# Soldann/MORB_SLAM

Hardware: AMD Instinct MI355X
Metric: stereo frames/sec ORB extract+match (752x480, 1200 feat = BASELINE configs[1]) (higher is better)
Workload: dtype u8; 1 GPU; BASELINE configs[1]: EuRoC-shaped stereo 752x480, 1200 feat: ORBextractor x2 + ComputeStereoMatches + ComputeBoW (synthetic k=10 L=6 vocabulary) + SearchByBoW vs previous frame; steps_in_flight=2, extract_streams=1, parallelism=frames dealt round-robin over 1 GPU(s)

## Files before the change

morb_slam_amd/csrc/matcher.hip:

```cpp
#include <hip/hip_runtime.h>

#include <algorithm>
#include <cstdlib>
#include <cstring>
#include <memory>
#include <vector>

#include "common.h"
#include "internal_abi.h"
#include "wave.h"
#include "extractor_internal.h"

using namespace morb;

namespace {

constexpr int TH_HIGH = 100, TH_LOW = 50, HISTO_LENGTH = 30;

struct Desc { uint32_t w[8]; };

__device__ __forceinline__ Desc load_desc(const uint8_t* p) {
  Desc d;
  const uint4* q = reinterpret_cast<const uint4*>(p);
  const uint4 a = q[0], b = q[1];
// ... 31 lines not shown
__global__ __launch_bounds__(256) void k_hamming_pairs(const uint8_t* __restrict__ a, const uint8_t* __restrict__ b, int n,
                                                       int* __restrict__ out) {
  const int i = blockIdx.x * 256 + threadIdx.x;
  if (i < n) out[i] = hamming(load_desc(a + (size_t)i * 32), load_desc(b + (size_t)i * 32));
}

__global__ __launch_bounds__(256) void k_knn2(const uint8_t* __restrict__ q, const int* __restrict__ nqv, int qPitch,
                                              const uint8_t* __restrict__ t, const int* __restrict__ ntv, int tPitch,
                                              const int* __restrict__ qOffv, const int* __restrict__ tOffv,
                                              int* __restrict__ idx, int* __restrict__ dist) {
  __shared__ uint4 tile[256 * 2];
  const int prob = blockIdx.y;
  const int qOff = qOffv ? qOffv[prob] : 0, tOff = tOffv ? tOffv[prob] : 0;
  const int nq = nqv[prob] - qOff, nt = ntv[prob] - tOff;
  const int i = blockIdx.x * 256 + threadIdx.x;
  const uint8_t* qb = q + ((size_t)prob * qPitch + qOff) * 32;
  const uint8_t* tb = t + ((size_t)prob * tPitch + tOff) * 32;
  if ((int)blockIdx.x * 256 >= nq) return;
  Desc d;
  if (i < nq) d = load_desc(qb + (size_t)i * 32);
  unsigned long long k1 = ~0ull, k2 = ~0ull;
  for (int j0 = 0; j0 < nt; j0 += 256) {
    const int j = j0 + threadIdx.x;
    if (j < nt) {
      const uint4* src = reinterpret_cast<const uint4*>(tb + (size_t)j * 32);
      tile[threadIdx.x * 2] = src[0];
      tile[threadIdx.x * 2 + 1] = src[1];
    }
    __syncthreads();
    const int m = nt - j0 < 256 ? nt - j0 : 256;
    if (i < nq) {
      for (int jj = 0; jj < m; ++jj) {
        const uint4 a = tile[jj * 2], b = tile[jj * 2 + 1];
        const int s = __popc(d.w[0] ^ a.x) + __popc(d.w[1] ^ a.y) + __popc(d.w[2] ^ a.z) + __popc(d.w[3] ^ a.w) +
                      __popc(d.w[4] ^ b.x) + __popc(d.w[5] ^ b.y) + __popc(d.w[6] ^ b.z) + __popc(d.w[7] ^ b.w);
        top2_insert(k1, k2, ((unsigned long long)s << 32) | (unsigned)(j0 + jj));
      }
    }
    __syncthreads();
  }
  if (i < nq) {
    const size_t o = ((size_t)prob * qPitch + i) * 2;
    idx[o] = k1 == ~0ull ? -1 : (int)(k1 & 0xFFFFFFFFu);
    dist[o] = k1 == ~0ull ? -1 : (int)(k1 >> 32);
    idx[o + 1] = k2 == ~0ull ? -1 : (int)(k2 & 0xFFFFFFFFu);
    dist[o + 1] = k2 == ~0ull ? -1 : (int)(k2 >> 32);
  }
}

__host__ __device__ inline int sm_lk_for(int nframes) { return nframes <= 2 ? 4 : nframes <= 8 ? 8 : nframes <= 32 ? 16 : 32; }
constexpr int SM_BAND = 16;
constexpr int SM_MAXB = 256;
struct StereoGeom {
  unsigned long long pyrOff[16], pyrImg[16];
  int pstride[16], w[16];
  float scale[16], invScale[16];
  int nRows;
};
struct RightKp { uint32_t band; float x; };
constexpr int SM_LIST = 4;
constexpr int SM_KQ = 8;
constexpr int SM_PCAP = 512;
constexpr int SM_PATCH = 11 * 12 + 11 * 24;
static_assert(4 * SM_PATCH <= SM_PCAP * 4, "four keypoints' patches reuse the pair list");
#define WAVE_SYNC() do { __builtin_amdgcn_fence(__ATOMIC_SEQ_CST, "workgroup"); __builtin_amdgcn_wave_barrier(); } while (0)
__device__ __forceinline__ uint32_t load_u32_unaligned(const uint8_t* p) { uint32_t v; __builtin_memcpy(&v, p, 4); return v; }

struct StereoRec { int band, list, bytes; };
__host__ __device__ inline StereoRec stereo_rec(int cap) {
  StereoRec r;
  r.band = (cap * (int)sizeof(RightKp) + 15) & ~15;
  r.list = r.band + (((SM_MAXB + 2) * 4 + 15) & ~15);
  r.bytes = r.list + ((SM_LIST * cap * 2 + 15) & ~15);
  return r;
}
__global__ __launch_bounds__(1024) void k_stereo_prep(const StereoGeom sg, const morb_keypoint* __restrict__ kps, const int* __restrict__ count,
                                                     int cap, uint8_t* __restrict__ rec) {
  extern __shared__ __align__(16) uint8_t smem[];
  const StereoRec ro = stereo_rec(cap);
  RightKp* tab = reinterpret_cast<RightKp*>(smem);
  int* bandStart = reinterpret_cast<int*>(smem + ro.band);
  uint16_t* list = reinterpret_cast<uint16_t*>(smem + ro.list);
  int* bandFill = reinterpret_cast<int*>(smem + ro.bytes);
  const int f = blockIdx.x, tid = threadIdx.x, lane = tid & 63, NT = blockDim.x;
  const int imgR = 2 * f + 1, NR = count[imgR];
  const int nRows = sg.nRows;
  const int nBands = (nRows + SM_BAND - 1) / SM_BAND;
  const bool banded = nBands <= SM_MAXB;
  for (int i = tid; i < SM_MAXB + 2; i += NT) { bandStart[i] = 0; if (i < SM_MAXB) bandFill[i] = 0; }
  __syncthreads();
  for (int iR = tid; iR < NR; iR += NT) {
    const morb_keypoint kpR = kps[(size_t)imgR * cap + iR];
    const float r = 2.0f * sg.scale[kpR.octave & 15];
    const int maxr = (int)ceilf(kpR.y + r), minr = (int)floorf(kpR.y - r);
    const int lo = min(max(minr, -4095), 4095) + 4096, hi = min(max(maxr, -4095), 4095) + 4096;
    RightKp t;
    t.band = (uint32_t)lo | ((uint32_t)hi << 14) | ((uint32_t)kpR.octave << 28); t.x = kpR.x;
    tab[iR] = t;
    if (banded && maxr >= 0 && minr < nRows)
      for (int bnd = max(minr, 0) / SM_BAND; bnd <= min(maxr, nRows - 1) / SM_BAND; ++bnd) atomicAdd(&bandStart[bnd + 1], 1);
  }
  __syncthreads();
  if (tid < 64) {
    int c[4], sum = 0;
#pragma unroll
    for (int k = 0; k < 4; ++k) { c[k] = bandStart[1 + tid * 4 + k]; sum += c[k]; }
    int inc = sum;
#pragma unroll
    for (int d = 1; d < 64; d <<= 1) { const int o = __shfl_up(inc, d, 64); if (lane >= d) inc += o; }
    int acc = inc - sum;
#pragma unroll
    for (int k = 0; k < 4; ++k) { acc += c[k]; bandStart[1 + tid * 4 + k] = acc; }
    if (tid == 63) bandStart[SM_MAXB + 1] = acc;
  }
  __syncthreads();
  const int listTotal = bandStart[SM_MAXB + 1];
  if (banded && listTotal <= SM_LIST * cap) {
    for (int iR = tid; iR < NR; iR += NT) {
      const RightKp t = tab[iR];
      const int minr = (int)(t.band & 0x3FFF) - 4096, maxr = (int)((t.band >> 14) & 0x3FFF) - 4096;
      if (maxr >= 0 && minr < nRows)
        for (int bnd = max(minr, 0) / SM_BAND; bnd <= min(maxr, nRows - 1) / SM_BAND; ++bnd)
          list[bandStart[bnd] + atomicAdd(&bandFill[bnd], 1)] = (uint16_t)iR;
    }
  }
  __syncthreads();
  const uint4* src = reinterpret_cast<const uint4*>(smem);
  uint4* dst = reinterpret_cast<uint4*>(rec + (size_t)f * ro.bytes);
  for (int i = tid; i < (ro.bytes >> 4); i += NT) dst[i] = src[i];
}

__global__ __launch_bounds__(256) void k_stereo_match(const StereoGeom sg, const uint8_t* __restrict__ pyr,
                                                      const morb_keypoint* __restrict__ kps,
                                                      const uint8_t* __restrict__ desc, const int* __restrict__ count,
                                                      int cap, float mbf, float mb,
                                                      float* __restrict__ uRight, float* __restrict__ depth,
                                                      int* __restrict__ sadDist, int SM_LK, const uint8_t* __restrict__ rec) {
  extern __shared__ __align__(16) uint8_t smem[];
  uint4* dLAll = reinterpret_cast<uint4*>(smem);
  unsigned long long* bestAll = reinterpret_cast<unsigned long long*>(dLAll + 4 * SM_KQ * 2);
  uint32_t* pairsAll = reinterpret_cast<uint32_t*>(bestAll + 4 * SM_KQ);
  uint8_t* recL = reinterpret_cast<uint8_t*>(pairsAll + 4 * SM_PCAP);
  const StereoRec ro = stereo_rec(cap);
  const RightKp* tab = reinterpret_cast<const RightKp*>(recL);
  const int* bandStart = reinterpret_cast<const int*>(recL + ro.band);
  const uint16_t* list = reinterpret_cast<const uint16_t*>(recL + ro.list);
  const int f = blockIdx.y, tid = threadIdx.x, lane = tid & 63, wv = tid >> 6;
  const int imgL = 2 * f, imgR = 2 * f + 1;
  const int NL = count[imgL], NR = count[imgR];
  const int iL0 = blockIdx.x * SM_LK;
  if (iL0 >= cap) return;
  const int nRows = sg.nRows;
  const int nBands = (nRows + SM_BAND - 1) / SM_BAND;
  const bool banded = nBands <= SM_MAXB;
  const uint8_t* recG = rec + (size_t)f * ro.bytes;
  const int listTotal = reinterpret_cast<const int*>(recG + ro.band)[SM_MAXB + 1];
  const bool useBands = banded && listTotal <= SM_LIST * cap;
  if (iL0 < NL) {
    const uint4* src = reinterpret_cast<const uint4*>(recG);
    uint4* dst = reinterpret_cast<uint4*>(recL);
    const int nTab = (NR * (int)sizeof(RightKp) + 15) >> 4, nBand = ((SM_MAXB + 2) * 4 + 15) >> 4, nList = useBands ? (listTotal * 2 + 15) >> 4 : 0;
    for (int i = tid; i < nTab; i += 256) dst[i] = src[i];
    for (int i = tid; i < nBand; i += 256) dst[(ro.band >> 4) + i] = src[(ro.band >> 4) + i];
    for (int i = tid; i < nList; i += 256) dst[(ro.list >> 4) + i] = src[(ro.list >> 4) + i];
  }
  __syncthreads();
#if defined(MORB_STEREO_STOP) && MORB_STEREO_STOP == 1
  return;
#endif
  const int KQ = SM_LK / 4;
  uint32_t* pairs = pairsAll + wv * SM_PCAP;
  uint4* dLs = dLAll + wv * (SM_KQ * 2);
  unsigned long long* bestL = bestAll + wv * SM_KQ;
  const uint64_t lt = lane == 0 ? 0ull : (~0ull >> (64 - lane));
  const float maxD = mbf / mb;
  float myX = 0.f, myY = 0.f;
  int myOct = 0;
  if (lane < KQ) {
    const int iL = iL0 + lane * 4 + wv;
    if (iL < NL) { const morb_keypoint k = kps[(size_t)imgL * cap + iL]; myX = k.x; myY = k.y; myOct = k.octave; }
  }
  if (lane < 2 * KQ) {
    const int iL = iL0 + (lane >> 1) * 4 + wv;
    uint4 v = make_uint4(0, 0, 0, 0);
    if (iL < NL) v = reinterpret_cast<const uint4*>(desc + ((size_t)imgL * cap + iL) * 32)[lane & 1];
    dLs[lane] = v;
  }
  if (lane < SM_KQ) bestL[lane] = ~0ull;
  WAVE_SYNC();

  auto flush = [&](int n) {
    WAVE_SYNC();
    for (int c0 = 0; c0 < n; c0 += 64) {
      const int c = c0 + lane;
      const bool act = c < n;
      const uint32_t pr = pairs[act ? c : n - 1];
      const int q = (int)(pr >> 16), jR = (int)(pr & 0xFFFFu);
      unsigned long long key = ~0ull;
      if (act) {
        Desc dL;
        const uint4 a = dLs[2 * q], b = dLs[2 * q + 1];
        dL.w[0] = a.x; dL.w[1] = a.y; dL.w[2] = a.z; dL.w[3] = a.w; dL.w[4] = b.x; dL.w[5] = b.y; dL.w[6] = b.z; dL.w[7] = b.w;
        const int d = hamming(dL, load_desc(desc + ((size_t)imgR * cap + jR) * 32));
        if (d < TH_HIGH) key = ((unsigned long long)d << 32) | (unsigned)jR;
      }
      if (cap <= 65536) {
        static_assert(SM_KQ <= 256 && TH_HIGH <= 256, "the packed key holds (SM_KQ - 1 - q) in 8 bits, a distance < TH_HIGH in 8 bits and the right index in 16");
        uint32_t ck = ((uint32_t)(SM_KQ - 1 - q) << 24) | (key == ~0ull ? 0xFFFFFFu : (((uint32_t)(key >> 32) << 16) | (uint32_t)(key & 0xFFFFu)));
        MORB_DPP_SCAN(ck, 0xFFFFFFFFu, morbwave::op_umin);
        const int qn = (int)(pairs[c + 1 < n ? c + 1 : n - 1] >> 16);
        const bool runEnd = act && (c == n - 1 || lane == 63 || qn != q);
        const uint32_t m24 = ck & 0xFFFFFFu;
        if (runEnd && m24 != 0xFFFFFFu) {
          const unsigned long long m = ((unsigned long long)(m24 >> 16) << 32) | (m24 & 0xFFFFu);
          if (m < bestL[q]) bestL[q] = m;
        }
      } else {
        const int qlo = __builtin_amdgcn_readfirstlane(q), qhi = __builtin_amdgcn_readlane(q, 63);
        for (int qq = qlo; qq <= qhi; ++qq) {
          const unsigned long long m = wave_min_u64(q == qq ? key : ~0ull);
          if (lane == 0 && m < bestL[qq]) bestL[qq] = m;
        }
      }
    }
    WAVE_SYNC();
  };
  {
    int n = 0;
    for (int q = 0; q < KQ; ++q) {
      const int iL = iL0 + q * 4 + wv;
      if (iL >= NL) break;
      const int levelL = __builtin_amdgcn_readlane(myOct, q);
      const float vL = __builtin_bit_cast(float, __builtin_amdgcn_readlane(__builtin_bit_cast(int, myY), q));
      const float uL = __builtin_bit_cast(float, __builtin_amdgcn_readlane(__builtin_bit_cast(int, myX), q));
      const int row = (int)vL;
      const float minU = uL - maxD, maxU = uL - 0.f;
      if (!(row >= 0 && row < nRows && !(maxU < 0))) continue;
      const int e0 = useBands ? bandStart[row / SM_BAND] : 0, e1 = useBands ? bandStart[row / SM_BAND + 1] : NR;
      for (int j0 = e0; j0 < e1; j0 += 64) {
        const int ei = j0 + lane;
        bool ok = false;
        int iR = 0;
        if (ei < e1) {
          iR = useBands ? (int)list[ei] : ei;
          const RightKp t = tab[iR];
          const int minr = (int)(t.band & 0x3FFF) - 4096, maxr = (int)((t.band >> 14) & 0x3FFF) - 4096, oct = (int)(t.band >> 28);
          ok = row >= minr && row <= maxr && !(oct < levelL - 1 || oct > levelL + 1) && t.x >= minU && t.x <= maxU;
        }
        const uint64_t m = __ballot(ok);
        if (ok) pairs[n + __popcll(m & lt)] = ((uint32_t)q << 16) | (uint32_t)iR;
        n += __popcll(m);
        if (n > SM_PCAP - 64) { flush(n); n = 0; }
      }
    }
    if (n) flush(n);
  }
#if defined(MORB_STEREO_STOP) && MORB_STEREO_STOP == 2
  return;
#endif
  bool cDo = false;
  float cUL = 0.f, cUR0 = 0.f;
  int cLvl = 0, cPs = 0;
  unsigned long long cOffL = 0, cOffR = 0;
  if (lane < KQ) {
    const int iL = iL0 + lane * 4 + wv;
    if (iL < NL) {
      const unsigned long long best = bestL[lane];
      const int bestDist = best == ~0ull ? TH_HIGH : (int)(best >> 32);
      if (bestDist < (TH_HIGH + TH_LOW) / 2) {
        const int bestIdxR = (int)(best & 0xFFFFFFFFu);
        const int levelL = myOct;
        const float vL = myY, uL = myX;
        const float uR0 = tab[bestIdxR].x;
        const float sf = sg.invScale[levelL & 15];
        const float scaleduL = roundf(uL * sf), scaledvL = roundf(vL * sf), scaleduR0 = roundf(uR0 * sf);
        const unsigned long long pyrOff = sg.pyrOff[levelL & 15], pyrImg = sg.pyrImg[levelL & 15];
        const int pstride = sg.pstride[levelL & 15], w = sg.w[levelL & 15];
        const float iniu = scaleduR0 + 5 - 5, endu = scaleduR0 + 5 + 5 + 1;
        if (!(iniu < 0 || endu >= (float)w)) {
          cDo = true; cUL = uL; cUR0 = scaleduR0; cLvl = levelL; cPs = pstride;
          cOffL = pyrOff + (size_t)imgL * pyrImg + (size_t)(kPyrPad + (int)scaledvL) * pstride + kPyrPad + (int)scaleduL;
          cOffR = pyrOff + (size_t)imgR * pyrImg + (size_t)(kPyrPad + (int)scaledvL) * pstride + kPyrPad + (int)scaleduR0;
        }
      }
    }
  }
  int pRow[2], pCol[2], pLds[2];
  bool pLeft[2], pAct[2];
#pragma unroll
  for (int j = 0; j < 2; ++j) {
    const int t = lane + 64 * j;
    pAct[j] = t < 99; pLeft[j] = t < 33;
    if (t < 33) {
      const int r = t / 3, c4 = (t - r * 3) * 4;
      pRow[j] = r - 5; pCol[j] = c4 - 5; pLds[j] = r * 12 + c4;
    } else {
      const int t2 = min(t, 98) - 33, r = t2 / 6, c4 = (t2 - r * 6) * 4;
      pRow[j] = r - 5; pCol[j] = c4 - 10; pLds[j] = 11 * 12 + r * 24 + c4;
    }
  }
  const uint64_t doMask = __ballot(cDo);
  const uint32_t cOffLlo = (uint32_t)cOffL, cOffLhi = (uint32_t)(cOffL >> 32), cOffRlo = (uint32_t)cOffR, cOffRhi = (uint32_t)(cOffR >> 32);
  uint8_t* patch = reinterpret_cast<uint8_t*>(pairs);
  int rS = -1, rInc = 0;
  float rD1 = 0.f, rD3 = 0.f;
  const int dy = min(lane & 15, 10);
  for (int q0 = 0; q0 < KQ; q0 += 4) {
    if (((doMask >> q0) & 15ull) == 0) continue;
    uint32_t pv[4][2];
#pragma unroll
    for (int k = 0; k < 4; ++k) {
      const int q = q0 + k;
      pv[k][0] = pv[k][1] = 0;
      if ((doMask >> q) & 1ull) {
        const unsigned long long oL = ((unsigned long long)(uint32_t)__builtin_amdgcn_readlane((int)cOffLhi, q) << 32) | (uint32_t)__builtin_amdgcn_readlane((int)cOffLlo, q);
        const unsigned long long oR = ((unsigned long long)(uint32_t)__builtin_amdgcn_readlane((int)cOffRhi, q) << 32) | (uint32_t)__builtin_amdgcn_readlane((int)cOffRlo, q);
        const int ps = __builtin_amdgcn_readlane(cPs, q);
#pragma unroll
        for (int j = 0; j < 2; ++j)
          if (pAct[j]) pv[k][j] = load_u32_unaligned(pyr + (pLeft[j] ? oL : oR) + (ptrdiff_t)pRow[j] * ps + pCol[j]);
      }
    }
    WAVE_SYNC();
#pragma unroll
    for (int k = 0; k < 4; ++k) {
      if (!((doMask >> (q0 + k)) & 1ull)) continue;
#pragma unroll
      for (int j = 0; j < 2; ++j)
        if (pAct[j]) *reinterpret_cast<uint32_t*>(patch + k * SM_PATCH + pLds[j]) = pv[k][j];
    }
    WAVE_SYNC();
#pragma unroll
    for (int k = 0; k < 4; ++k) {
      const int q = q0 + k;
      if (!((doMask >> q) & 1ull)) continue;
      const uint8_t* Lp = patch + k * SM_PATCH;
      const uint8_t* Rp = Lp + 11 * 12;
      const uint32_t l0 = *reinterpret_cast<const uint32_t*>(Lp + dy * 12), l1 = *reinterpret_cast<const uint32_t*>(Lp + dy * 12 + 4),
                     l2 = *reinterpret_cast<const uint32_t*>(Lp + dy * 12 + 8) & 0x00FFFFFFu;
      uint32_t bestKey = 0xFFFFFFFFu;
      int sums[12];
#pragma unroll
      for (int r = 0; r < 3; ++r) {
        const int sh = min(r * 4 + (lane >> 4), 10);
        const uint8_t* rp = Rp + dy * 24 + (sh & ~3);
        const uint32_t w0 = *reinterpret_cast<const uint32_t*>(rp), w1 = *reinterpret_cast<const uint32_t*>(rp + 4),
                       w2 = *reinterpret_cast<const uint32_t*>(rp + 8), w3 = *reinterpret_cast<const uint32_t*>(rp + 12);
        const uint32_t bsh = (uint32_t)(sh & 3);
        const uint32_t r0 = __builtin_amdgcn_alignbyte(w1, w0, bsh), r1 = __builtin_amdgcn_alignbyte(w2, w1, bsh),
                       r2 = __builtin_amdgcn_alignbyte(w3, w2, bsh) & 0x00FFFFFFu;
        int sv = (int)__builtin_amdgcn_sad_u8(l2, r2, __builtin_amdgcn_sad_u8(l1, r1, __builtin_amdgcn_sad_u8(l0, r0, 0u)));
        if ((lane & 15) > 10) sv = 0;
        sv += __builtin_amdgcn_update_dpp(0, sv, 0x111, 0xf, 0xf, true);
        sv += __builtin_amdgcn_update_dpp(0, sv, 0x112, 0xf, 0xf, true);
        sv += __builtin_amdgcn_update_dpp(0, sv, 0x114, 0xf, 0xf, true);
        sv += __builtin_amdgcn_update_dpp(0, sv, 0x118, 0xf, 0xf, true);
#pragma unroll
        for (int j = 0; j < 4; ++j) {
          sums[r * 4 + j] = __builtin_amdgcn_readlane(sv, 16 * j + 15);
          if (r * 4 + j < 11) {
            const uint32_t key = ((uint32_t)sums[r * 4 + j] << 4) | (uint32_t)(r * 4 + j);
            bestKey = key < bestKey ? key : bestKey;
          }
        }
      }
      const int bestS = (int)(bestKey >> 4), bi = (int)(bestKey & 15u);
      int s1 = 0, s3 = 0;
#pragma unroll
      for (int i = 0; i < 11; ++i) { s1 = (i == bi - 1) ? sums[i] : s1; s3 = (i == bi + 1) ? sums[i] : s3; }
      if (lane == q) { rS = bestS; rInc = bi - 5; rD1 = (float)s1; rD3 = (float)s3; }
    }
  }
  if (lane < KQ) {
    const int iL = iL0 + lane * 4 + wv;
    if (iL < cap) {
      float outU = -1.0f, outD = -1.0f;
      int outS = -1;
      if (cDo) {
        const int bestinc = rInc, bestS = rS;
        if (!(bestinc == -5 || bestinc == 5)) {
          const float dist1 = rD1, dist2 = (float)bestS, dist3 = rD3;
          const float deltaR = (dist1 - dist3) / (2.0f * (dist1 + dist3 - 2.0f * dist2));
          if (!(deltaR < -1 || deltaR > 1)) {
            float bestuR = sg.scale[cLvl & 15] * ((float)cUR0 + (float)bestinc + deltaR);
            float disparity = cUL - bestuR;
            if (disparity >= 0.f && disparity < maxD) {
              if (disparity <= 0) {
                disparity = 0.01f;
                bestuR = (float)((double)cUL - 0.01);
              }
              outD = mbf / disparity;
              outU = bestuR;
              outS = bestS;
            }
          }
        }
      }
      const size_t o = (size_t)f * cap + iL;
      uRight[o] = outU; depth[o] = outD; sadDist[o] = outS;
    }
  }
}

constexpr int SMED_V = 8;
template <int SMED_WAVES>
__global__ __launch_bounds__(64 * SMED_WAVES) void k_stereo_median(const int* __restrict__ count, int cap, float* __restrict__ uRight,
                                                       float* __restrict__ depth, const int* __restrict__ sadDist) {
  constexpr int NT = 64 * SMED_WAVES;
  const int f = blockIdx.x, tid = threadIdx.x;
  const int NL = count[2 * f];
  const size_t o = (size_t)f * cap;
  const bool inRegs = NL <= NT * SMED_V;
  int dv[SMED_V];
#pragma unroll
  for (int j = 0; j < SMED_V; ++j) { const int i = tid + j * NT; dv[j] = (inRegs && i < NL) ? sadDist[o + i] : -1; }
  int n = 0;
  if (inRegs) {
#pragma unroll
    for (int j = 0; j < SMED_V; ++j) n += dv[j] >= 0 ? 1 : 0;
  } else {
    for (int i = tid; i < NL; i += NT) n += sadDist[o + i] >= 0 ? 1 : 0;
  }
  __shared__ int red[2][SMED_WAVES];
  int phase = 0;
  auto blockSum = [&](int v) -> int {
    v = wave_sum(v);
    if ((tid & 63) == 0) red[phase][tid >> 6] = v;
    __syncthreads();
    int t = 0;
#pragma unroll
    for (int q = 0; q < SMED_WAVES; ++q) t += red[phase][q];
    phase ^= 1;
    return t;
  };
  const int total = blockSum(n);
  if (total == 0) return;
  const int k = total / 2;
  int lo = 0, hi = 121 * 255;
  while (lo < hi) {
    const int mid = (lo + hi) >> 1;
    int c = 0;
    if (inRegs) {
#pragma unroll
      for (int j = 0; j < SMED_V; ++j) c += (dv[j] >= 0 && dv[j] <= mid) ? 1 : 0;
    } else {
      for (int i = tid; i < NL; i += NT) { const int d = sadDist[o + i]; c += (d >= 0 && d <= mid) ? 1 : 0; }
    }
    c = blockSum(c);
    if (c > k) hi = mid; else lo = mid + 1;
  }
  const float median = (float)lo;
  const float thDist = 1.5f * 1.4f * median;
  if (inRegs) {
#pragma unroll
    for (int j = 0; j < SMED_V; ++j) {
      const int i = tid + j * NT;
      if (dv[j] >= 0 && !((float)dv[j] < thDist)) { uRight[o + i] = -1; depth[o + i] = -1; }
    }
  } else {
    for (int i = tid; i < NL; i += NT) {
      const int d = sadDist[o + i];
      if (d >= 0 && !((float)d < thDist)) { uRight[o + i] = -1; depth[o + i] = -1; }
    }
  }
}

__device__ __forceinline__ int quad_sum(int v) {
  v += __builtin_amdgcn_update_dpp(0, v, 0xB1, 0xF, 0xF, false);
  v += __builtin_amdgcn_update_dpp(0, v, 0x4E, 0xF, 0xF, false);
  return v;
}
__global__ __launch_bounds__(256) void k_bow_transform(const uint8_t* __restrict__ feat, const int* __restrict__ count,
                                                       int cap, const uint8_t* __restrict__ nodeDesc,
                                                       const int* __restrict__ firstChild, int k, int L, int levelsup,
                                                       int* __restrict__ wordId, int* __restrict__ nodeId,
                                                       const int* __restrict__ childCount) {
  const int img = blockIdx.y, t = blockIdx.x * 256 + threadIdx.x, i = t >> 2, sub = t & 3;
  if (i >= cap) return;
  const size_t o = (size_t)img * cap + i;
  if (i >= count[img]) { if (sub == 0) { wordId[o] = -1; nodeId[o] = -1; } return; }
  const uint2 d = *reinterpret_cast<const uint2*>(feat + o * 32 + sub * 8);
  const uint8_t* nd = nodeDesc + sub * 8;
  const int nid_level = L - levelsup;
  int final_id = 0, level = 0, nid = 0;
  do {
    ++level;
    const int c0 = firstChild[final_id];
    const int nc = childCount ? childCount[final_id] : k;
    int best = c0, bestd = 0x7fffffff;
    constexpr int CH = 5;
    for (int cb = c0; cb < c0 + nc; cb += CH) {
      uint2 tc[CH];
#pragma unroll
      for (int j = 0; j < CH; ++j) tc[j] = *reinterpret_cast<const uint2*>(nd + (size_t)min(cb + j, c0 + nc - 1) * 32);
#pragma unroll
      for (int j = 0; j < CH; ++j) {
        const int dd = quad_sum(__popc(d.x ^ tc[j].x) + __popc(d.y ^ tc[j].y));
        if (dd < bestd) { bestd = dd; best = min(cb + j, c0 + nc - 1); }
      }
    }
    final_id = best;
    if (level == nid_level) nid = final_id;
  } while (firstChild[final_id] >= 0);
  if (sub == 0) { wordId[o] = final_id; nodeId[o] = nid; }
}

constexpr int BT_K = 10, BT_N1 = BT_K, BT_N2 = BT_K * BT_K, BT_N3 = BT_K * BT_K * BT_K, BT_SLOTS = BT_N1 + BT_N2 + BT_N3;
template <int NLV> struct BtLds {
  static constexpr int SLOTS = NLV == 3 ? BT_SLOTS : BT_N1 + BT_N2;
  uint2 desc[SLOTS][4];
  int id[SLOTS];
  int fc[SLOTS];
  uint16_t nc[SLOTS];
};
template <int NLV>
__global__ __launch_bounds__(256) void k_bow_transform_lds(const uint8_t* __restrict__ feat, const int* __restrict__ count, int cap, int nimg,
                                                           const uint8_t* __restrict__ nodeDesc, const int* __restrict__ firstChild, int k,
                                                           int L, int levelsup, int* __restrict__ wordId, int* __restrict__ nodeId,
                                                           const int* __restrict__ childCount) {
  extern __shared__ __align__(16) uint8_t btRaw[];
  BtLds<NLV>& S = *reinterpret_cast<BtLds<NLV>*>(btRaw);
  const int tid = threadIdx.x;
  const int fc0 = firstChild[0], nc0 = childCount ? childCount[0] : k;
  auto stage = [&](int slot, int parentFc, int parentNc, int j) {
    int id = -1, fc = -1, nc = 0;
    if (parentFc >= 0 && j < parentNc) {
      id = parentFc + j;
      fc = firstChild[id];
      nc = fc >= 0 ? (childCount ? childCount[id] : k) : 0;
      const uint4* src = reinterpret_cast<const uint4*>(nodeDesc + (size_t)id * 32);
      const uint4 a = src[0], b = src[1];
      S.desc[slot][0] = make_uint2(a.x, a.y); S.desc[slot][1] = make_uint2(a.z, a.w);
      S.desc[slot][2] = make_uint2(b.x, b.y); S.desc[slot][3] = make_uint2(b.z, b.w);
    }
    S.id[slot] = id; S.fc[slot] = fc; S.nc[slot] = (uint16_t)min(nc, 0xFFFF);
  };
  if (tid < BT_N1) stage(tid, nc0 <= BT_K ? fc0 : -1, nc0, tid);
  __syncthreads();
  if (tid < BT_N2) { const int a = tid / BT_K; stage(BT_N1 + tid, S.nc[a] <= BT_K ? S.fc[a] : -1, S.nc[a], tid % BT_K); }
  __syncthreads();
  if (NLV == 3) for (int t = tid; t < BT_N3; t += 256) { const int ab = t / BT_K; stage(BT_N1 + BT_N2 + t, S.nc[BT_N1 + ab] <= BT_K ? S.fc[BT_N1 + ab] : -1, S.nc[BT_N1 + ab], t % BT_K); }
  __syncthreads();
  const int sub = tid & 3, nid_level = L - levelsup;
  const int chunksPerImg = (cap + 63) / 64, nChunks = chunksPerImg * nimg;
  const uint8_t* nd = nodeDesc + sub * 8;
  for (int ch = blockIdx.x; ch < nChunks; ch += gridDim.x) {
    const int img = ch / chunksPerImg, i = (ch - img * chunksPerImg) * 64 + (tid >> 2);
    if (i >= cap) continue;
    const size_t o = (size_t)img * cap + i;
    if (i >= count[img]) { if (sub == 0) { wordId[o] = -1; nodeId[o] = -1; } continue; }
    const uint2 d = *reinterpret_cast<const uint2*>(feat + o * 32 + sub * 8);
    int final_id = 0, level = 0, nid = 0;
    int slotBase = 0, nc = nc0, path = 0;
    bool leaf = fc0 < 0;
#pragma unroll
    for (int lv = 0; lv < NLV; ++lv) {
      if (leaf || nc > BT_K) break;
      ++level;
      int best = 0, bestd = 0x7fffffff;
      for (int j = 0; j < nc; ++j) {
        const uint2 tc = S.desc[slotBase + j][sub];
        const int dd = quad_sum(__popc(d.x ^ tc.x) + __popc(d.y ^ tc.y));
        if (dd < bestd) { bestd = dd; best = j; }
      }
      const int slot = slotBase + best;
      final_id = S.id[slot];
      if (level == nid_level) nid = final_id;
      leaf = S.fc[slot] < 0;
      nc = S.nc[slot];
      path = path * BT_K + best;
      slotBase = (lv == 0 ? BT_N1 : BT_N1 + BT_N2) + path * BT_K;
    }
    while (!leaf) {
      ++level;
      const int c0 = firstChild[final_id];
      const int ncg = childCount ? childCount[final_id] : k;
      int best = c0, bestd = 0x7fffffff;
      constexpr int CH = 5;
      for (int cb = c0; cb < c0 + ncg; cb += CH) {
        uint2 tc[CH];
#pragma unroll
        for (int j = 0; j < CH; ++j) tc[j] = *reinterpret_cast<const uint2*>(nd + (size_t)min(cb + j, c0 + ncg - 1) * 32);
#pragma unroll
        for (int j = 0; j < CH; ++j) {
          const int dd = quad_sum(__popc(d.x ^ tc[j].x) + __popc(d.y ^ tc[j].y));
          if (dd < bestd) { bestd = dd; best = min(cb + j, c0 + ncg - 1); }
        }
      }
      final_id = best;
      if (level == nid_level) nid = final_id;
      leaf = firstChild[final_id] < 0;
    }
    if (sub == 0) { wordId[o] = final_id; nodeId[o] = nid; }
  }
}

__global__ __launch_bounds__(1024) void k_bow_sort(const int* __restrict__ node, const int* __restrict__ count, int cap,
                                                   int P, unsigned long long* __restrict__ sorted) {
  extern __shared__ unsigned long long skeys[];
  const int img = blockIdx.x, tid = threadIdx.x, NT = blockDim.x;
  const int n = count[img];
  if (n == 0) {
    for (int i = tid; i < cap; i += NT) sorted[(size_t)img * cap + i] = ~0ull;
    return;
  }
  for (int i = tid; i < P; i += NT) {
    unsigned long long k = ~0ull;
    if (i < n) {
      const int nd = node[(size_t)img * cap + i];
      if (nd >= 0) k = ((unsigned long long)(unsigned)nd << 32) | (unsigned)i;
    }
    skeys[i] = k;
  }
  __syncthreads();
  const bool onePass = P / 2 <= NT;
  for (int k = 2; k <= P; k <<= 1)
    for (int j = k >> 1; j > 0; j >>= 1) {
      for (int l = tid; l < P / 2; l += NT) {
        const int i = ((l & ~(j - 1)) << 1) | (l & (j - 1)), ixj = i | j;
        const unsigned long long a = skeys[i], b = skeys[ixj];
        const bool up = (i & k) == 0;
        if ((a > b) == up) { skeys[i] = b; skeys[ixj] = a; }
      }
      const int jn = j > 1 ? j >> 1 : k;
      if (onePass && jn < 64 && j < 64) { __builtin_amdgcn_fence(__ATOMIC_SEQ_CST, "wavefront"); __builtin_amdgcn_wave_barrier(); }
      else __syncthreads();
    }
  for (int i = tid; i < cap; i += NT) sorted[(size_t)img * cap + i] = i < P ? skeys[i] : ~0ull;
}

#ifdef MORB_FAST_TIMING
__device__ unsigned long long g_bowTrace[16384 * 4];
#define BOW_MARK(k) do { if (lane == 0 && bw_ < 16384) g_bowTrace[bw_ * 4 + (k)] = wall_clock64(); } while (0)
#else
#define BOW_MARK(k)
#endif
constexpr int BM_NB = 25;
constexpr int BM_FJ = 4;
__device__ __forceinline__ unsigned wave_min_u32(unsigned v) { return morbwave::min_u32(v); }
__global__ __launch_bounds__(256) void k_bow_match(const unsigned long long* __restrict__ sortedKF,
                                                   const unsigned long long* __restrict__ sortedF,
                                                   const int* __restrict__ nKFv, const int* __restrict__ nFv, int cap,
                                                   const uint8_t* __restrict__ descKF, const uint8_t* __restrict__ hasMP,
                                                   const morb_keypoint* __restrict__ kpsKF,
                                                   const uint8_t* __restrict__ descF, const morb_keypoint* __restrict__ kpsF,
                                                   const int* __restrict__ kfImg, const int* __restrict__ fImg,
                                                   float nnratio, int* __restrict__ matchF, int* __restrict__ binF,
                                                   const int* __restrict__ nLeftv,
                                                   const uint8_t* __restrict__ hasMP2, const int* __restrict__ nValidv,
                                                   int* __restrict__ matched2) {
  extern __shared__ __align__(16) unsigned long long bowLds[];
#ifdef MORB_FAST_TIMING
  const int bw_ = (blockIdx.y * gridDim.x + blockIdx.x) * 4 + (threadIdx.x >> 6);
  if ((threadIdx.x & 63) == 0 && bw_ < 16384) g_bowTrace[bw_ * 4] = wall_clock64();
#endif
  unsigned long long* sk = bowLds;
  unsigned long long* sf = bowLds + cap;
  const int pair = blockIdx.y, tid = threadIdx.x, lane = tid & 63, wv = tid >> 6;
  const int ik = kfImg[pair], jf = fImg[pair];
  const int nKF = nKFv[ik], nF = nFv[jf];
  const bool fish = nLeftv != nullptr && nLeftv[pair] >= 0;
  const int nLeft = fish ? nLeftv[pair] : 0x7fffffff;
  const bool kfkf = hasMP2 != nullptr;
  const int nValid1 = (kfkf && nValidv) ? nValidv[ik] : 0x7fffffff, nValid2 = (kfkf && nValidv) ? nValidv[jf] : 0x7fffffff;
  const int thLow = kfkf ? TH_LOW - 1 : TH_LOW;
  {
    const unsigned long long* gk = sortedKF + (size_t)ik * cap;
    const unsigned long long* gf = sortedF + (size_t)jf * cap;
    for (int i0 = 0; i0 < cap; i0 += 256 * 4) {
      unsigned long long a[4], b[4];
#pragma unroll
      for (int k = 0; k < 4; ++k) {
        const int i = i0 + k * 256 + tid;
        a[k] = i < nKF ? gk[i] : ~0ull;
// ... 653 lines not shown
```

Measured before the change: 141,200 frames/s.

## Compute stereo SAD for four keypoints at once with packed 16-bit sums

The stereo refinement now gives each 16-lane row of the wave its own keypoint from the group of four. Each lane evaluates all 11 disparity shifts, packing two 16-bit SAD totals per dword via sad_u8/sad_hi_u8, and reduces the six packed words with DPP. This replaces the serial per-keypoint loop of three rounds, each ending in a chain of readlanes. The row totals are stored in LDS behind the patch buffers, and each owning lane then does its own argmin and neighbour lookup after the loop. This removes serial readlane and argmin work per keypoint. It relies on SAD totals fitting in 16 bits and adds LDS stores and reads.

Result: no change. 140,100 frames/s (-0.8%).

```diff
diff --git a/morb_slam_amd/csrc/matcher.hip b/morb_slam_amd/csrc/matcher.hip
--- a/morb_slam_amd/csrc/matcher.hip
+++ b/morb_slam_amd/csrc/matcher.hip
@@ -357,9 +357,9 @@
   const uint64_t doMask = __ballot(cDo);
   const uint32_t cOffLlo = (uint32_t)cOffL, cOffLhi = (uint32_t)(cOffL >> 32), cOffRlo = (uint32_t)cOffR, cOffRhi = (uint32_t)(cOffR >> 32);
   uint8_t* patch = reinterpret_cast<uint8_t*>(pairs);
-  int rS = -1, rInc = 0;
-  float rD1 = 0.f, rD3 = 0.f;
-  const int dy = min(lane & 15, 10);
+  uint32_t* sadSums = reinterpret_cast<uint32_t*>(patch + 4 * SM_PATCH);
+  static_assert(4 * SM_PATCH + SM_KQ * 6 * 4 <= SM_PCAP * 4, "the SAD totals sit behind the four patches in the dead pair list");
+  const int prow = lane >> 4, dy = min(lane & 15, 10);
   for (int q0 = 0; q0 < KQ; q0 += 4) {
     if (((doMask >> q0) & 15ull) == 0) continue;
     uint32_t pv[4][2];
@@ -385,46 +385,56 @@
         if (pAct[j]) *reinterpret_cast<uint32_t*>(patch + k * SM_PATCH + pLds[j]) = pv[k][j];
     }
     WAVE_SYNC();
-#pragma unroll
-    for (int k = 0; k < 4; ++k) {
-      const int q = q0 + k;
-      if (!((doMask >> q) & 1ull)) continue;
-      const uint8_t* Lp = patch + k * SM_PATCH;
-      const uint8_t* Rp = Lp + 11 * 12;
-      const uint32_t l0 = *reinterpret_cast<const uint32_t*>(Lp + dy * 12), l1 = *reinterpret_cast<const uint32_t*>(Lp + dy * 12 + 4),
-                     l2 = *reinterpret_cast<const uint32_t*>(Lp + dy * 12 + 8) & 0x00FFFFFFu;
-      uint32_t bestKey = 0xFFFFFFFFu;
-      int sums[12];
-#pragma unroll
-      for (int r = 0; r < 3; ++r) {
-        const int sh = min(r * 4 + (lane >> 4), 10);
-        const uint8_t* rp = Rp + dy * 24 + (sh & ~3);
-        const uint32_t w0 = *reinterpret_cast<const uint32_t*>(rp), w1 = *reinterpret_cast<const uint32_t*>(rp + 4),
-                       w2 = *reinterpret_cast<const uint32_t*>(rp + 8), w3 = *reinterpret_cast<const uint32_t*>(rp + 12);
+    {
+      const uint32_t* Lp = reinterpret_cast<const uint32_t*>(patch + prow * SM_PATCH + dy * 12);
+      const uint32_t* Rp = reinterpret_cast<const uint32_t*>(patch + prow * SM_PATCH + 11 * 12 + dy * 24);
+      const uint32_t l0 = Lp[0], l1 = Lp[1], l2 = Lp[2] & 0x00FFFFFFu;
+      uint32_t w[6];
+#pragma unroll
+      for (int i = 0; i < 6; ++i) w[i] = Rp[i];
+      uint32_t pk[6];
+#pragma unroll
+      for (int sh = 0; sh < 11; ++sh) {
+        const int b = sh >> 2;
         const uint32_t bsh = (uint32_t)(sh & 3);
-        const uint32_t r0 = __builtin_amdgcn_alignbyte(w1, w0, bsh), r1 = __builtin_amdgcn_alignbyte(w2, w1, bsh),
-                       r2 = __builtin_amdgcn_alignbyte(w3, w2, bsh) & 0x00FFFFFFu;
-        int sv = (int)__builtin_amdgcn_sad_u8(l2, r2, __builtin_amdgcn_sad_u8(l1, r1, __builtin_amdgcn_sad_u8(l0, r0, 0u)));
-        if ((lane & 15) > 10) sv = 0;
+        const uint32_t r0 = bsh ? __builtin_amdgcn_alignbyte(w[b + 1], w[b], bsh) : w[b],
+                       r1 = bsh ? __builtin_amdgcn_alignbyte(w[b + 2], w[b + 1], bsh) : w[b + 1],
+                       r2 = (bsh ? __builtin_amdgcn_alignbyte(w[b + 3], w[b + 2], bsh) : w[b + 2]) & 0x00FFFFFFu;
+        if (!(sh & 1)) pk[sh >> 1] = __builtin_amdgcn_sad_u8(l2, r2, __builtin_amdgcn_sad_u8(l1, r1, __builtin_amdgcn_sad_u8(l0, r0, 0u)));
+        else pk[sh >> 1] = __builtin_amdgcn_sad_hi_u8(l2, r2, __builtin_amdgcn_sad_hi_u8(l1, r1, __builtin_amdgcn_sad_hi_u8(l0, r0, pk[sh >> 1])));
+      }
+#pragma unroll
+      for (int j = 0; j < 6; ++j) {
+        int sv = (int)pk[j];
         sv += __builtin_amdgcn_update_dpp(0, sv, 0x111, 0xf, 0xf, true);
         sv += __builtin_amdgcn_update_dpp(0, sv, 0x112, 0xf, 0xf, true);
         sv += __builtin_amdgcn_update_dpp(0, sv, 0x114, 0xf, 0xf, true);
         sv += __builtin_amdgcn_update_dpp(0, sv, 0x118, 0xf, 0xf, true);
-#pragma unroll
-        for (int j = 0; j < 4; ++j) {
-          sums[r * 4 + j] = __builtin_amdgcn_readlane(sv, 16 * j + 15);
-          if (r * 4 + j < 11) {
-            const uint32_t key = ((uint32_t)sums[r * 4 + j] << 4) | (uint32_t)(r * 4 + j);
-            bestKey = key < bestKey ? key : bestKey;
-          }
-        }
-      }
-      const int bestS = (int)(bestKey >> 4), bi = (int)(bestKey & 15u);
-      int s1 = 0, s3 = 0;
-#pragma unroll
-      for (int i = 0; i < 11; ++i) { s1 = (i == bi - 1) ? sums[i] : s1; s3 = (i == bi + 1) ? sums[i] : s3; }
-      if (lane == q) { rS = bestS; rInc = bi - 5; rD1 = (float)s1; rD3 = (float)s3; }
-    }
+        pk[j] = (uint32_t)sv;
+      }
+      if ((lane & 15) == 10) {
+#pragma unroll
+        for (int j = 0; j < 6; ++j) sadSums[(q0 + prow) * 6 + j] = pk[j];
+      }
+    }
+  }
+  WAVE_SYNC();
+  int rS = -1, rInc = 0;
+  float rD1 = 0.f, rD3 = 0.f;
+  if (cDo) {
+    const uint32_t* sp = sadSums + lane * 6;
+    uint32_t bestKey = 0xFFFFFFFFu;
+#pragma unroll
+    for (int j = 0; j < 6; ++j) {
+      const uint32_t v = sp[j];
+      const uint32_t ke = ((v & 0xFFFFu) << 4) | (uint32_t)(2 * j), ko = ((v >> 16) << 4) | (uint32_t)(2 * j + 1);
+      bestKey = ke < bestKey ? ke : bestKey;
+      if (2 * j + 1 < 11) bestKey = ko < bestKey ? ko : bestKey;
+    }
+    const int bi = (int)(bestKey & 15u);
+    const uint16_t* sh16 = reinterpret_cast<const uint16_t*>(sp);
+    rS = (int)(bestKey >> 4); rInc = bi - 5;
+    rD1 = (float)sh16[max(bi - 1, 0)]; rD3 = (float)sh16[min(bi + 1, 10)];
   }
   if (lane < KQ) {
     const int iL = iL0 + lane * 4 + wv;
```
